# sloisel/MultiGridBarrier.jl

Hardware: AMD Instinct MI355X
Metric: Newton iters/sec + wall-clock to converge, 2D P2 p-Laplace L=9 (higher is better)
Workload: dtype f64

## Files before the change

### multigridbarrier.jl_amd/csrc/mf_big_inv.hpp

```cpp
#pragma once
#include "mf_device.hpp"
#include "mf_big_subst.hpp"

namespace mgbhip {
namespace {

constexpr int BIGI_THREADS = 1024;

#include "ldlt32.hpp"

__device__ __forceinline__ void block_ldlt32(double (*Dn)[NB + 1], double* dq, int nb, int tid, int32_t* __restrict__ status) {
    block_ldlt32_mfma(Dn, dq, nb, tid, status);
}
__device__ __forceinline__ void block_inverse32_sel(const double (*Ls)[NB + 1], double (*Wv)[NB + 1], double (*Tm)[17], int tid) {
    block_inverse32_mfma(Ls, Wv, Tm, tid);
}

__device__ __forceinline__ void slice_transform(double (*P)[ST + 1], double (*Pout)[ST + 1], double (*P2)[ST + 1],
                                                const double (*Wv)[NB + 1], const double* rd, int lane, int wave) {
    const int fr = lane & 15, fk = lane >> 4;
    const int rr = 16 * wave + fr;
    double4_t acc0 = {0.0, 0.0, 0.0, 0.0}, acc1 = {0.0, 0.0, 0.0, 0.0};
#pragma unroll
    for (int kk = 0; kk < NB / 4; ++kk) {
        const double a = P[4 * kk + fk][rr];
        if (kk < 4) acc0 = __builtin_amdgcn_mfma_f64_16x16x4f64(Wv[fr][4 * kk + fk], a, acc0, 0, 0, 0);
        acc1 = __builtin_amdgcn_mfma_f64_16x16x4f64(Wv[16 + fr][4 * kk + fk], a, acc1, 0, 0, 0);
    }
#pragma unroll
    for (int r = 0; r < 4; ++r) {
        const int q0 = fk + 4 * r, q1 = 16 + fk + 4 * r;
        Pout[q0][rr] = acc0[r];
        Pout[q1][rr] = acc1[r];
        if (P2) {
            P2[q0][rr] = acc0[r] * rd[q0];
            P2[q1][rr] = acc1[r] * rd[q1];
        }
    }
}

#ifdef MGB_STEP_PROBE
#define PROBE(i) do { __builtin_amdgcn_sched_barrier(0); __builtin_amdgcn_s_waitcnt(0); if (is_la && blockIdx.y == 0 && tid == 0 && j0 == 64 && gridDim.y == 1 && F.k > 400) g_probe[i] = wall_clock64(); if (!is_la && blockIdx.x == 0 && blockIdx.y == 0 && tid == 0 && j0 == 64 && gridDim.y == 1 && F.k > 400) g_probe[16 + i] = wall_clock64(); __builtin_amdgcn_s_waitcnt(0); __builtin_amdgcn_sched_barrier(0); } while (0)
#else
#define PROBE(i) do { } while (0)
#endif

__global__ __launch_bounds__(256, 3) void mf_big_step(const FrontDev* __restrict__ fr, int32_t first, int j0,
                                                   double* __restrict__ arena, double* __restrict__ dscr,
                                                   double* __restrict__ dvec, int32_t* __restrict__ status,
                                                   int do_diag) {
    __shared__ double Wv[NB][NB + 1];
    __shared__ double Dn[NB][NB + 1];
    __shared__ double Tm[16][17];
    __shared__ double dq[NB], rdq[NB];
    __shared__ double Pa[NB][ST + 1];
    __shared__ double Pb[NB][ST + 1];
    const FrontDev F = fr[first + blockIdx.y];
    const int m = F.m, k = F.k;
    if (j0 >= k) return;
    const int nb = min(NB, k - j0);
    const int j1 = j0 + nb;
    const int T = (m - j1 + ST - 1) / ST;
    const int tid = threadIdx.x, lane = tid & 63, wave = tid >> 6;
    double* W = arena + F.F_off;
    double* slot = dscr + ((int64_t)blockIdx.y * 2 + ((j0 / NB) & 1)) * (NB * NB);
    const bool is_la = blockIdx.x == gridDim.x - 1;
    int ti = 0, tj = 0;
    if (!is_la) {
        const int lin = blockIdx.x;
        ti = (int)((sqrt(8.0 * lin + 1.0) - 1.0) * 0.5);
        while ((ti + 1) * (ti + 2) / 2 <= lin) ++ti;
        while (ti * (ti + 1) / 2 > lin) --ti;
        tj = lin - ti * (ti + 1) / 2;
        if (ti >= T) return;
    }
    const bool look = j1 < k;
    const int nbn = look ? min(NB, k - j1) : 0;
    const int rbase = is_la ? j1 : j1 + ti * ST, cbase = j1 + tj * ST;
    PROBE(0);
#ifdef MGB_STEP_PROBE
    if (is_la && blockIdx.y == 0 && tid == 0 && j0 == 64 && gridDim.y == 1 && F.k > 400) g_probe[34] = clock64();
#endif
    const int fr16 = lane & 15, fk = lane >> 4;

    double pa[NB * ST / 256], pb[NB * ST / 256];
#pragma unroll
    for (int u = 0; u < NB * ST / 256; ++u) {
        const int i = tid + 256 * u, rr = i % ST, q = i / ST;
        const int r = rbase + rr, c = cbase + rr;
        const bool rin = is_la ? (rr < nbn) : (r < m);
        pa[u] = (q < nb && rin) ? W[r + (int64_t)(j0 + q) * m] : 0.0;
        pb[u] = (!is_la && ti != tj && q < nb && c < m) ? W[c + (int64_t)(j0 + q) * m] : 0.0;
    }
    double cw[4][4];
    if (!is_la) {
#pragma unroll
        for (int tb = 0; tb < 4; ++tb)
#pragma unroll
            for (int r = 0; r < 4; ++r) {
                const int row = rbase + 16 * wave + fr16, col = cbase + 16 * tb + fk + 4 * r;
                cw[tb][r] = (row < m && col < m && row >= col) ? W[row + (int64_t)col * m] : 0.0;
            }
    } else {
#pragma unroll
        for (int t = 0; t < 4; ++t) {
            const int i = tid + 256 * t, rr = i % NB, c = i / NB;
            cw[0][t] = (look && rr >= c && rr < nbn) ? W[(j1 + rr) + (int64_t)(j1 + c) * m] : 0.0;
        }
    }
    if (do_diag) {
        for (int i = tid; i < NB * NB; i += 256) {
            const int rr = i % NB, c = i / NB;
            Dn[rr][c] = (rr >= c && rr < nb) ? W[(j0 + rr) + (int64_t)(j0 + c) * m] : 0.0;
        }
        __syncthreads();
        block_ldlt32(Dn, dq, nb, tid, is_la ? status : nullptr);
        block_inverse32_sel(Dn, Wv, Tm, tid);
    } else {
        for (int i = tid; i < NB * NB; i += 256) {
            const int rr = i % NB, c = i / NB;
            const double v = (rr >= c && rr < nb) ? slot[rr + NB * c] : 0.0;
            Wv[rr][c] = (rr > c) ? v : (rr == c ? 1.0 : 0.0);
            if (rr == c) dq[rr] = (rr < nb) ? v : 1.0;
        }
    }
#pragma unroll
    for (int u = 0; u < NB * ST / 256; ++u) {
        const int i = tid + 256 * u, rr = i % ST, q = i / ST;
        Pa[q][rr] = pa[u];
        Pb[q][rr] = pb[u];
    }
    __syncthreads();
    PROBE(1);
    if (tid < NB) rdq[tid] = 1.0 / dq[tid];
    if (is_la ? T == 0 : blockIdx.x == 0) {
        {
            const int rt = wave & 1, ct = wave >> 1;
            if (ct <= rt) {
                double4_t accm = {0.0, 0.0, 0.0, 0.0};
#pragma unroll
                for (int kk = 0; kk < NB / 4; ++kk) {
                    const int kq = 4 * kk + fk;
                    accm = __builtin_amdgcn_mfma_f64_16x16x4f64(kq < nb ? Wv[kq][16 * ct + fr16] / dq[kq] : 0.0, Wv[kq][16 * rt + fr16], accm, 0, 0, 0);
                }
#pragma unroll
                for (int r = 0; r < 4; ++r) {
                    const int row = 16 * rt + fr16, col = 16 * ct + fk + 4 * r;
                    if (row < nb && col < row) W[(j0 + col) + (int64_t)(j0 + row) * m] = accm[r];
                    else if (row < nb && col == row) dvec[F.idx_off + j0 + row] = accm[r];
                }
            }
        }
    }
    if (is_la && !look) return;
    __syncthreads();
    PROBE(2);
    if (is_la) {
        if (wave < 2) slice_transform(Pa, Pa, Pb, Wv, rdq, lane, wave);
        __syncthreads();
        PROBE(3);
        {
            const int rt = wave & 1, ct = wave >> 1;
            double4_t accd = {0.0, 0.0, 0.0, 0.0};
#pragma unroll
            for (int kk = 0; kk < NB / 4; ++kk)
                accd = __builtin_amdgcn_mfma_f64_16x16x4f64(Pb[4 * kk + fk][16 * ct + fr16], Pa[4 * kk + fk][16 * rt + fr16],
                                                            accd, 0, 0, 0);
#pragma unroll
            for (int r = 0; r < 4; ++r) {
                const int rr = 16 * rt + fr16, c = 16 * ct + fk + 4 * r;
                Dn[rr][c] = -accd[r];
            }
        }
        __syncthreads();
#pragma unroll
        for (int t = 0; t < 4; ++t) {
            const int i = tid + 256 * t, rr = i % NB, c = i / NB;
            Dn[rr][c] = (rr >= c && rr < nbn) ? cw[0][t] + Dn[rr][c] : 0.0;
        }
        __syncthreads();
        double* nslot = dscr + ((int64_t)blockIdx.y * 2 + ((j1 / NB) & 1)) * (NB * NB);
        PROBE(4);
#ifdef MGB_STEP_PROBE
        double sv[4];
        for (int t = 0; t < 4; ++t) { const int i = tid + 256 * t; sv[t] = Dn[i % NB][i / NB]; }
        __syncthreads();
        __builtin_amdgcn_sched_barrier(0);
        if (is_la && blockIdx.y == 0 && tid == 0 && j0 == 64 && gridDim.y == 1 && F.k > 400) { g_probe[32] = clock64(); g_probe[36] = wall_clock64(); }
        __builtin_amdgcn_sched_barrier(0);
        block_ldlt32(Dn, dq, nbn, tid, nullptr);
        __builtin_amdgcn_sched_barrier(0);
        if (is_la && blockIdx.y == 0 && tid == 0 && j0 == 64 && gridDim.y == 1 && F.k > 400) { g_probe[33] = clock64(); g_probe[37] = wall_clock64(); }
        __builtin_amdgcn_sched_barrier(0);
        for (int t = 0; t < 4; ++t) { const int i = tid + 256 * t; Dn[i % NB][i / NB] = sv[t]; }
        __syncthreads();
        __builtin_amdgcn_sched_barrier(0);
        if (is_la && blockIdx.y == 0 && tid == 0 && j0 == 64 && gridDim.y == 1 && F.k > 400) { g_probe[38] = clock64(); g_probe[44] = wall_clock64(); }
        __builtin_amdgcn_sched_barrier(0);
#endif
        block_ldlt32(Dn, dq, nbn, tid, status);
#ifdef MGB_STEP_PROBE
        __builtin_amdgcn_sched_barrier(0);
        if (is_la && blockIdx.y == 0 && tid == 0 && j0 == 64 && gridDim.y == 1 && F.k > 400) { g_probe[39] = clock64(); g_probe[45] = wall_clock64(); }
        __builtin_amdgcn_sched_barrier(0);
#endif
        PROBE(5);
        block_inverse32_sel(Dn, Wv, Tm, tid);
        PROBE(6);
        for (int i = tid; i < NB * NB; i += 256) {
            const int rr = i % NB, c = i / NB;
            if (rr >= c && rr < nbn) nslot[rr + NB * c] = (rr == c) ? dq[rr] : Wv[rr][c];
        }
        PROBE(7);
#ifdef MGB_STEP_PROBE
        if (is_la && blockIdx.y == 0 && tid == 0 && j0 == 64 && gridDim.y == 1 && F.k > 400) g_probe[35] = clock64();
#endif
        return;
    }
    if (ti == tj) {
        slice_transform(Pa, Pa, Pb, Wv, rdq, lane, wave);
    } else {
        slice_transform(Pa, Pa, nullptr, Wv, rdq, lane, wave);
        {
            const int rr = 16 * wave + fr16;
            double4_t acc0 = {0.0, 0.0, 0.0, 0.0}, acc1 = {0.0, 0.0, 0.0, 0.0};
#pragma unroll
            for (int kk = 0; kk < NB / 4; ++kk) {
                const double a = Pb[4 * kk + fk][rr];
                if (kk < 4) acc0 = __builtin_amdgcn_mfma_f64_16x16x4f64(Wv[fr16][4 * kk + fk], a, acc0, 0, 0, 0);
                acc1 = __builtin_amdgcn_mfma_f64_16x16x4f64(Wv[16 + fr16][4 * kk + fk], a, acc1, 0, 0, 0);
            }
#pragma unroll
            for (int r = 0; r < 4; ++r) {
                const int q0 = fk + 4 * r, q1 = 16 + fk + 4 * r;
                Pb[q0][rr] = acc0[r] * rdq[q0];
                Pb[q1][rr] = acc1[r] * rdq[q1];
            }
        }
    }
    __syncthreads();
    PROBE(3);
    double4_t acc[4];
#pragma unroll
    for (int tb = 0; tb < 4; ++tb) acc[tb] = double4_t{0.0, 0.0, 0.0, 0.0};
#pragma unroll
    for (int kk = 0; kk < NB / 4; ++kk) {
        const double s = Pa[4 * kk + fk][16 * wave + fr16];
#pragma unroll
        for (int tb = 0; tb < 4; ++tb) {
            if (ti == tj && tb > wave) continue;
            acc[tb] = __builtin_amdgcn_mfma_f64_16x16x4f64(Pb[4 * kk + fk][16 * tb + fr16], s, acc[tb], 0, 0, 0);
        }
    }
    const int nskip = (blockIdx.x == 0 && look) ? nbn : 0;
#pragma unroll
    for (int tb = 0; tb < 4; ++tb)
#pragma unroll
        for (int r = 0; r < 4; ++r) {
            const int row = rbase + 16 * wave + fr16, col = cbase + 16 * tb + fk + 4 * r;
            if (row < m && col < m && row >= col && !(row - j1 < nskip && col - j1 < nskip))
                W[row + (int64_t)col * m] = cw[tb][r] - acc[tb][r];
        }
    PROBE(4);
}

__global__ __launch_bounds__(256) void mf_tri_pack(int m, const double* __restrict__ F, double* __restrict__ packed, int unpack,
                                                   double* __restrict__ Fout) {
    const int c = blockIdx.x;
    if (c >= m) return;
    const int64_t base = (int64_t)c * m - ((int64_t)c * (c - 1)) / 2;
    for (int r = c + threadIdx.x; r < m; r += 256) {
        if (unpack) Fout[r + (int64_t)c * m] = packed[base + (r - c)];
        else packed[base + (r - c)] = F[r + (int64_t)c * m];
    }
}

__global__ __launch_bounds__(256) void mf_big_diag0(const FrontDev* __restrict__ fr, int32_t first,
                                                    const double* __restrict__ arena, double* __restrict__ dscr,
                                                    int32_t* __restrict__ status) {
    __shared__ double Wv[NB][NB + 1];
    __shared__ double Dn[NB][NB + 1];
    __shared__ double Tm[16][17];
    __shared__ double dq[NB];
    const FrontDev F = fr[first + blockIdx.x];
    const int m = F.m, nb = min(NB, F.k), tid = threadIdx.x;
    const double* W = arena + F.F_off;
    for (int i = tid; i < NB * NB; i += 256) {
        const int rr = i % NB, c = i / NB;
        Dn[rr][c] = (rr >= c && rr < nb) ? W[rr + (int64_t)c * m] : 0.0;
    }
    __syncthreads();
    block_ldlt32(Dn, dq, nb, tid, status);
    block_inverse32_sel(Dn, Wv, Tm, tid);
    double* slot = dscr + (int64_t)blockIdx.x * 2 * (NB * NB);
    for (int i = tid; i < NB * NB; i += 256) {
        const int rr = i % NB, c = i / NB;
        if (rr >= c && rr < nb) slot[rr + NB * c] = (rr == c) ? dq[rr] : Wv[rr][c];
    }
}

__global__ __launch_bounds__(256) void mf_big_gather(const FrontDev* __restrict__ fr, int32_t first,
                                                     const GatherRec* __restrict__ grec, const int32_t* __restrict__ gmap,
                                                     const int32_t* __restrict__ a_src,
                                                     const int32_t* __restrict__ a_dst,
                                                     const int32_t* __restrict__ a_colptr,
                                                     const double* __restrict__ Hval, double* __restrict__ arena,
                                                     double* __restrict__ dscr, int32_t* __restrict__ status, int with_diag,
                                                     int ct ) {
    const FrontDev F = fr[first + blockIdx.y];
    const GatherRec G = grec[blockIdx.y];
    const int m = F.m;
    const int32_t* mp = gmap + G.map_off;
    if (with_diag && blockIdx.x == gridDim.x - 1) {
        __shared__ double Wv[NB][NB + 1];
        __shared__ double Dn[NB][NB + 1];
        __shared__ double Tm[16][17];
// ... 517 lines not shown
                for (int t = 0; t < 4; ++t) v += pa[ps][t].a * zr[2 * t] + pa[ps][t].b * zr[2 * t + 1];
                v += quad_perm_f64<0xB1>(v);
                v += quad_perm_f64<0x4E>(v);
                if (cp == 0) gl[q] += v;
            }
        }
        for (int q = cq + 2 * CPP; q - cq < j0; q += CPP) {
            const double* Aq = Fm + (int64_t)min(q, j0 - 1) * m + j0 + 2 * cp;
            D2 a[4];
#pragma unroll
            for (int t = 0; t < 4; ++t) {
                if (nb == NB) a[t] = *reinterpret_cast<const D2*>(Aq + 8 * t);
                else {
                    const int o = 2 * cp + 8 * t;
                    a[t].a = Aq[min(o, nb - 1) - 2 * cp];
                    a[t].b = Aq[min(o + 1, nb - 1) - 2 * cp];
                }
            }
            double v = 0.0;
#pragma unroll
            for (int t = 0; t < 4; ++t) v += a[t].a * zr[2 * t] + a[t].b * zr[2 * t + 1];
            v += quad_perm_f64<0xB1>(v);
            v += quad_perm_f64<0x4E>(v);
            if (cp == 0 && q < j0) gl[q] += v;
        }
        if (j0 == 256) BP(7);
        __syncthreads();
    }
    BP(9);
}

inline void launch_big_assemble(const FactorArgs& a, const MfLaunch& L, bool with_diag) {
    if (big_assembly_kind(L) != MF_ASM_GATHER) {
        launch_big_assemble_cols(a, L);
        return;
    }
    if (a.grec) {
        const int ct = big_gather_ct(L, a.gather_ct);
        const dim3 ga((L.max_m + ct - 1) / ct + (with_diag ? 1 : 0), L.count);
        hipLaunchKernelGGL(mf_big_gather, ga, dim3(256), big_gather_lds(L), a.st, a.fr, L.first, a.grec + L.grec_first, a.gmap,
                           a.a_src, a.a_dst, a.a_colptr, a.values, a.arena, a.dscr, a.status, with_diag ? 1 : 0, ct);
        return;
    }
    dim3 ga = big_assemble_grid(L);
    const int ct = CT;
    if (with_diag) ga.x += 1;
    hipLaunchKernelGGL(mf_big_gather_lds, ga, dim3(256), big_gather_lds(L), a.st, a.fr, L.first, a.children, a.rel, a.a_src, a.a_dst,
                       a.a_colptr, a.values, a.arena, L.max_m, a.dscr, a.status, with_diag ? 1 : 0, ct);
}

inline void launch_big_diag0(const FactorArgs& a, const MfLaunch& L, int nfronts) {
    hipLaunchKernelGGL(mf_big_diag0, dim3(nfronts), dim3(256), 0, a.st, a.fr, L.first, a.arena, a.dscr, a.status);
}
inline void launch_inv_steps(const FactorArgs& a, const MfLaunch& L, int nfronts, bool diag_in_step0) {
    for (int j0 = 0; j0 < L.max_k; j0 += NB) {
        const int rem = L.max_m - j0;
        const int T = std::max(0, (rem - 1 + ST - 1) / ST);
        const dim3 gs(T * (T + 1) / 2 + 1, nfronts);
        hipLaunchKernelGGL(mf_big_step, gs, dim3(256), 0, a.st, a.fr, L.first, j0, a.arena, a.dscr, a.dvec, a.status,
                           (j0 == 0 && diag_in_step0) ? 1 : 0);
    }
}

inline void launch_tri_pack(int m, double* F, double* packed, bool unpack, hipStream_t st) {
    hipLaunchKernelGGL(mf_tri_pack, dim3(m), dim3(256), 0, st, m, unpack ? (const double*)nullptr : F, packed, unpack ? 1 : 0,
                       unpack ? F : (double*)nullptr);
}

inline size_t fwd_inv_lds(int max_m) {
    return (size_t)(((max_m + 1) & ~1) + NB * (NB + 1) + 2 * NB + BIGI_THREADS) * sizeof(double);
}
inline size_t bwd_inv_lds(int max_m, int max_k) {
    return (size_t)(((max_m + 1) & ~1) + ((max_k + 1) & ~1) + NB * (NB + 1) + 2 * NB + (max_m + 1) / 2) * sizeof(double);
}
inline void launch_fwd_inv(const SolveArgs& a, const MfLaunch& L) {
    hipLaunchKernelGGL(mf_fwd_inv, dim3(L.count), dim3(BIGI_THREADS), fwd_inv_lds(L.max_m), a.st, a.fr, L.first, a.front_idx,
                       a.ug_ptr, a.ug_src, a.arena, a.dvec, a.b, a.y, a.uvec);
}
inline void launch_bwd_inv(const SolveArgs& a, const MfLaunch& L) {
    hipLaunchKernelGGL(mf_bwd_inv, dim3(L.count), dim3(BIGI_THREADS), bwd_inv_lds(L.max_m, L.max_k), a.st, a.fr, L.first,
                       a.front_idx, a.arena, a.dvec, a.y, a.x);
}

}
}
```

### multigridbarrier.jl_amd/csrc/mf_launch_plan.hpp

```cpp
#pragma once
#include <algorithm>
#include <cstdint>
#include <cstdlib>
#include <vector>

#include "mf_analysis.hpp"

namespace mgbhip {

struct MfLaunch {
    int32_t first, count;
    int32_t cls;
    int32_t max_m, max_k;
    int32_t max_child = 0;
    bool tiny = false;
    bool wave = false;
    bool inv = false;
    bool iface = false;
    int32_t grec_first = -1;
};

constexpr int BIG_INV_MAX_M = 7000;
constexpr int GATHER_MAX_CHILD = 8;
constexpr int BIG_DIAG0_MIN_COUNT = 24;

struct MfSwitches {
    bool no_geo;
    bool old_big;
    bool merge_groups;
    bool packed_leaves;
    bool wave_small;
    int64_t inv_min_n;
    int64_t wave_min_n;
    bool gather_lds_maps;
    int gather_ct;
    static MfSwitches from_env() {
        auto on = [](const char* name) { const char* e = getenv(name); return e && e[0] == '1'; };
        auto num = [](const char* name, long long dflt) { const char* e = getenv(name); return e ? atoll(e) : dflt; };
        return {on("MGBHIP_NO_GEO"), on("MGBHIP_OLD_BIG"), !on("MGBHIP_NO_MERGE_GROUPS"), !on("MGBHIP_NO_PACKED_LEAVES"),
                !on("MGBHIP_NO_WAVE_SMALL"), num("MGBHIP_INV_MIN_N", 1024), num("MGBHIP_WAVE_MIN_N", 0),
                on("MGBHIP_GATHER_LDS_MAPS"), (int)num("MGBHIP_GATHER_CT", 0)};
    }
};

using LevelLaunches = std::vector<std::vector<MfLaunch>>;

inline MfLaunch launch_of_range(const MfPlan& plan, MfLaunch L, int32_t first, int32_t count) {
    L.first = first; L.count = count;
    L.max_m = 0; L.max_k = 0; L.max_child = 0;
    for (int32_t t = first; t < first + count; ++t) {
        L.max_m = std::max(L.max_m, plan.fronts[t].m);
        L.max_k = std::max(L.max_k, plan.fronts[t].k);
        L.max_child = std::max(L.max_child, plan.fronts[t].nchild);
    }
    return L;
}

inline void merge_straggler_groups(const MfPlan& plan, std::vector<MfLaunch>& G) {
    auto absorb = [&](size_t into, size_t from) {
        MfLaunch& A = G[into];
        const MfLaunch& B = G[from];
        A.first = B.first;
        A.count += B.count;
        A.max_k = std::max(A.max_k, B.max_k);
        A.max_child = std::max(A.max_child, B.max_child);
        G.erase(G.begin() + (long)from);
    };
    if (G.size() >= 2 && G.back().cls == 0 && G.back().inv) {
        int64_t lds_count = 0;
        bool ok = true;
        for (size_t g = 0; g + 1 < G.size(); ++g) { lds_count += G[g].count; ok = ok && !G[g].tiny && plan.fronts[G[g].first].m > 32; }
        if (ok && lds_count <= G.back().count)
            while (G.size() >= 2) absorb(G.size() - 1, G.size() - 2);
    }
    for (size_t g = 0; g + 1 < G.size();) {
        const bool next_lds = G[g + 1].cls != 0;
        if (next_lds && !G[g].tiny && (G[g].count < 256 || 4 * (int64_t)G[g].count < G[g + 1].count)) absorb(g + 1, g);
        else ++g;
    }
}

inline void split_interface_front(const MfPlan& plan, LevelLaunches& levels, bool inv_allowed) {
    const int32_t q = plan.iface_front;
    for (auto& G : levels) {
        for (size_t g = 0; g < G.size(); ++g) {
            const MfLaunch L = G[g];
            if (q < L.first || q >= L.first + L.count) continue;
            std::vector<MfLaunch> out;
            if (q > L.first) out.push_back(launch_of_range(plan, L, L.first, q - L.first));
            MfLaunch I = launch_of_range(plan, L, q, 1);
            I.cls = 0; I.tiny = false; I.wave = false; I.iface = true;
            I.inv = (I.max_m <= BIG_INV_MAX_M && inv_allowed);
            out.push_back(I);
            if (q + 1 < L.first + L.count) out.push_back(launch_of_range(plan, L, q + 1, L.first + L.count - q - 1));
// ... 99 lines not shown
inline MfAssembly big_assembly_kind(const MfLaunch& L) {
    if (L.cls) return MF_ASM_NONE;
    if (L.max_child < 1 || L.max_child > GATHER_MAX_CHILD || big_gather_lds(L) > 40 * 1024) return MF_ASM_COLS;
    return MF_ASM_GATHER;
}
inline MfBlock0 big_block0_kind(const MfLaunch& L, bool inv) {
    if (L.cls || !inv) return MF_B0_NA;
    if (!L.iface && big_assembly_kind(L) == MF_ASM_GATHER) return MF_B0_GATHER;
    return (L.iface || L.count >= BIG_DIAG0_MIN_COUNT) ? MF_B0_DIAG0 : MF_B0_STEP0;
}
inline int backward_small_kmax(const MfLaunch& L) { return L.max_k <= 8 ? 8 : (L.max_k <= 16 ? 16 : 0); }

constexpr int GATHER_MIN_WGS = 768;
inline int big_gather_ct(const MfLaunch& L, int forced) {
    if (forced == 8 || forced == 16 || forced == 32) return forced;
    int ct = 8;
    while (ct < 32 && (int64_t)L.count * ((L.max_m + 2 * ct - 1) / (2 * ct)) >= GATHER_MIN_WGS) ct *= 2;
    return ct;
}

struct GatherRec {
    int64_t map_off;
    int64_t base[GATHER_MAX_CHILD];
    int32_t ld[GATHER_MAX_CHILD];
    int32_t bs[GATHER_MAX_CHILD];
};

inline void build_gather_maps(const MfPlan& plan, LevelLaunches& levels, std::vector<GatherRec>& recs, std::vector<int32_t>& gmap) {
    recs.clear();
    gmap.clear();
    for (auto& lev : levels)
        for (auto& L : lev) {
            L.grec_first = -1;
            if (L.count == 0 || big_assembly_kind(L) != MF_ASM_GATHER) continue;
            L.grec_first = (int32_t)recs.size();
            for (int32_t q = L.first; q < L.first + L.count; ++q) {
                const Front& f = plan.fronts[q];
                GatherRec R{};
                R.map_off = (int64_t)gmap.size();
                gmap.resize(gmap.size() + (size_t)f.nchild * (size_t)f.m, -1);
                for (int32_t c = 0; c < f.nchild; ++c) {
                    const Front& ch = plan.fronts[plan.children[f.child_off + c]];
                    R.base[c] = ch.F_off + (int64_t)ch.k * ch.m + ch.k;
                    R.ld[c] = ch.m;
                    R.bs[c] = ch.m - ch.k;
                    int32_t* mp = gmap.data() + R.map_off + (int64_t)c * f.m;
                    for (int32_t j = 0; j < ch.m - ch.k; ++j) mp[plan.rel[ch.rel_off + j]] = j;
                }
                recs.push_back(R);
            }
        }
}

constexpr int MF_LAUNCH_ROW = 16;
inline int64_t launch_rows(const LevelLaunches& levels, const LevelLaunches& solves, bool leaf_packed, bool robust,
                           int32_t* out, int64_t cap) {
    int64_t n = 0;
    for (size_t l = 0; l < levels.size(); ++l) {
        int32_t bwd = 0;
        for (auto& S : solves[l])
            if (S.cls && !S.tiny) { const int km = backward_small_kmax(S); bwd = km == 8 ? MF_BWD_K8 : (km == 16 ? MF_BWD_K16 : MF_BWD_GENERAL); }
        for (auto& L : levels[l]) {
            if (n < cap && out) {
                const bool inv = L.inv && !robust;
                int32_t* r = out + n * MF_LAUNCH_ROW;
                r[0] = (int32_t)l; r[1] = L.first; r[2] = L.count; r[3] = L.cls; r[4] = L.max_m; r[5] = L.max_k; r[6] = L.max_child;
                r[7] = L.tiny; r[8] = L.wave; r[9] = inv; r[10] = L.iface; r[11] = L.tiny && leaf_packed;
                r[12] = big_assembly_kind(L); r[13] = big_block0_kind(L, inv); r[14] = (L.cls && !L.tiny) ? bwd : (int32_t)MF_BWD_NA; r[15] = 0;
            }
            ++n;
        }
    }
    return n;
}

}
```

### multigridbarrier.jl_amd/csrc/mf_numeric.hip

```cpp
#include <hip/hip_runtime.h>

#include <cstdio>

#include <algorithm>
#include <cstdlib>

#include "../../include/mgbhip.h"
#include "mf_solver.hpp"
#include "mf_device.hpp"
#include "mf_small.hpp"
#include "mf_big_subst.hpp"
#include "mf_big_inv.hpp"

namespace mgbhip {

namespace {

int32_t query_lds_cap() {
    if (hipFuncSetAttribute((const void*)mf_factor_small<8, true>, hipFuncAttributeMaxDynamicSharedMemorySize,
                            (int)factor_small_lds(128)) == hipSuccess)
        return 128;
    (void)hipGetLastError();
    return 88;
}
// ... 108 lines not shown
        const double one = 1.0;
        d_one.upload(&one, 1, st);
        MGB_HIP_CHECK(hipStreamSynchronize(st));
    }
    d_tbig.alloc(plan.front_idx.size() ? plan.front_idx.size() : 1);
    d_tsol.alloc(plan.front_idx.size() ? plan.front_idx.size() : 1);
    d_dvec.alloc(plan.front_idx.size() ? plan.front_idx.size() : 1);
    d_status.alloc(2);
    d_status.zero(st);
}

void MfSolver::analyze(int64_t n, const int32_t* rowptr, const int32_t* colidx, hipStream_t st,
                       const double* coords, int dim, bool protect_peeled, const int32_t* top, int64_t ntop) {
    const MfSwitches sw = MfSwitches::from_env();
    MfOptions opt;
    opt.protect_peeled = protect_peeled;
    opt.top = top;
    opt.ntop = ntop;
    opt.border = true;
    mf_analyze(n, rowptr, colidx, opt, plan, sw.no_geo ? nullptr : coords, dim);
    const int32_t nf = (int32_t)plan.fronts.size();
    std::vector<FrontDev> fd(nf);
    for (int32_t i = 0; i < nf; ++i) {
        const Front& f = plan.fronts[i];
        fd[i] = FrontDev{f.k, f.m, f.nchild, f.a_cnt, f.F_off, f.idx_off, f.u_off, f.child_off, f.rel_off, f.a_off, f.acol_off, -1, 0, 0};
    }
    upload_plan(st);

    lds_cap = query_lds_cap();
    const bool inv_ok = !sw.old_big && query_inv_optin();
    level_launches = classify_launches(plan, lds_cap, inv_ok, sw);
    level_solves = merge_level_solves(level_launches);
    uses_inv = false;
    const std::vector<char> on_big_path = fronts_on_big_path(plan, level_launches);
    int32_t max_big = 1;
    for (auto& lev : level_launches)
        for (auto& L : lev) {
            uses_inv = uses_inv || L.inv;
            if (!L.cls) max_big = std::max(max_big, L.count);
        }
    d_dscr.alloc((size_t)max_big * 2 * NB * NB);

    std::vector<int64_t> ug_ptr, ug_src;
    build_gather_lists(plan, on_big_path, fd, ug_ptr, ug_src);
    leaf_packed = sw.packed_leaves && pack_leaf_fronts(plan, level_launches, on_big_path, fd);
    d_ug_ptr.upload(ug_ptr, st);
    d_ug_src.upload(ug_src, st);
    std::vector<GatherRec> grec;
    std::vector<int32_t> gmap;
    if (!sw.gather_lds_maps) build_gather_maps(plan, level_launches, grec, gmap);
    gather_ct = sw.gather_ct;
    if (grec.empty()) { d_grec.release(); d_gmap.release(); }
    else { d_grec.upload(grec, st); d_gmap.upload(gmap, st); }
    d_fronts.upload(fd, st);
    h_fronts = fd;
    h_a_dst = remap_a_dst(plan, level_launches);
    d_a_dst.upload(h_a_dst, st);
    if (const char* e = getenv("MGBHIP_DEBUG"); e && atoi(e) >= 2) dump_plan(plan, level_launches);
    analyzed = true;
    MGB_HIP_CHECK(hipStreamSynchronize(st));
}

void MfSolver::set_direct_map(const int32_t* value_map, int64_t nnz, int64_t tail_base, hipStream_t st) {
    std::vector<int32_t> as(plan.a_src.size());
    for (size_t t = 0; t < as.size(); ++t) {
        const int64_t src = plan.a_src[t];
        const int64_t v = src < nnz ? (int64_t)value_map[src] : tail_base + (src - nnz);
        MGB_REQUIRE(v < (int64_t)INT32_MAX, "direct value index exceeds 32 bits");
        as[t] = (int32_t)v;
    }
    d_a_src_direct.upload(as, st);
    MGB_HIP_CHECK(hipStreamSynchronize(st));
}

void MfSolver::factor(const double* d_values, hipStream_t st, StageTimers* timers, bool direct, bool condensed) {
    MGB_REQUIRE(!direct || d_a_src_direct.n > 0, "MfSolver::factor: no direct value map");
    MGB_REQUIRE(!condensed || (direct && condensed_ok), "MfSolver::factor: condensed leaves are not enabled");
    MGB_REQUIRE(analyzed, "MfSolver::factor before analyze");
    const FactorArgs a{condensed ? d_fronts_c.p : d_fronts.p, d_children.p, d_rel.p,
                       condensed ? d_a_src_c.p : (direct ? d_a_src_direct.p : d_a_src.p), condensed ? d_a_dst_c.p : d_a_dst.p,
                       condensed ? d_a_colptr_c.p : d_a_colptr.p, d_values, d_arena.p, d_dscr.p, d_dvec.p, d_status.p, st,
                       d_grec.n ? d_grec.p : nullptr, d_gmap.p, gather_ct};
    if (timers) timers->begin("factor");
    factored_inv = !robust;
    if (!status_zero) MGB_HIP_CHECK(hipMemsetAsync(d_status.p, 0, sizeof(int32_t), st));
    status_zero = false;
    factored_condensed = condensed;
    int lvno = -1;
    for (auto& lev : level_launches) {
        LevelScope lvscope(timers, "fac", ++lvno);
        for (auto& L : lev) {
            if (L.count == 0) continue;
            if (condensed && lvno == 0) continue;
            if (L.tiny) launch_factor_tiny(a, L);
            else if (L.wave && L.cls <= 32) launch_factor_wave<32>(a, L);
            else if (L.wave) launch_factor_wave<48>(a, L);
            else if (L.cls) launch_factor_small(a, L);
            else {
                const bool inv = L.inv && !robust;
                const MfBlock0 b0 = big_block0_kind(L, inv);
                MGB_REQUIRE(!L.iface || (bool)iface_reduce, "MfSolver: interface front without a reduction hook");
                launch_big_assemble(a, L, b0 == MF_B0_GATHER);
                if (L.iface) {
                    const Front& fi = plan.fronts[L.first];
                    const int64_t tri = (int64_t)fi.m * (fi.m + 1) / 2;
                    d_ifpack.ensure((size_t)tri);
                    launch_tri_pack(fi.m, d_arena.p + fi.F_off, d_ifpack.p, false, st);
                    iface_reduce(d_ifpack.p, tri);
                    launch_tri_pack(fi.m, d_arena.p + fi.F_off, d_ifpack.p, true, st);
                }
                if (inv) {
                    if (b0 == MF_B0_DIAG0) launch_big_diag0(a, L, L.count);
                    launch_inv_steps(a, L, L.count, b0 == MF_B0_STEP0);
                } else
                    launch_subst_steps(a, L, L.count);
            }
        }
    }
    MGB_HIP_CHECK(hipGetLastError());
    if (timers) timers->end();
}

void MfSolver::solve(const double* d_b, double* d_x, hipStream_t st, StageTimers* timers) {
    MGB_REQUIRE(analyzed, "MfSolver::solve before analyze");
    if (timers) timers->begin("trisolve");
    const size_t n = (size_t)plan.n;
    MGB_HIP_CHECK(hipMemcpyAsync(d_bx.p, d_b, n * sizeof(double), hipMemcpyDeviceToDevice, st));
    MGB_HIP_CHECK(hipMemsetAsync(d_bx.p + n, 0, sizeof(double), st));
    forward_pass(d_bx.p, st, timers);
    backward_pass(d_xx.p, st, timers);
    MGB_HIP_CHECK(hipMemcpyAsync(d_x, d_xx.p, n * sizeof(double), hipMemcpyDeviceToDevice, st));
    MGB_HIP_CHECK(hipGetLastError());
    if (timers) timers->end();
}

void MfSolver::solve_border(double* d_x_np1, hipStream_t st, StageTimers* timers) {
    MGB_REQUIRE(analyzed, "MfSolver::solve_border before analyze");
    if (timers) timers->begin("trisolve");
    const size_t n = (size_t)plan.n;
    if (!y_zero) {
        MGB_HIP_CHECK(hipMemsetAsync(d_y.p, 0, n * sizeof(double), st));
        y_zero = true;
    }
    if (!y_border_one) {
        MGB_HIP_CHECK(hipMemcpyAsync(d_y.p + n, d_one.p, sizeof(double), hipMemcpyDeviceToDevice, st));
        y_border_one = true;
    }
    backward_pass(d_x_np1, st, timers);
    MGB_HIP_CHECK(hipGetLastError());
    if (timers) timers->end();
}

void MfSolver::forward_pass(const double* d_b, hipStream_t st, StageTimers* timers) {
    y_border_one = false;
    y_zero = false;
    const SolveArgs a = solve_args(d_b, nullptr, st);
    int lvno = -1;
    for (auto& lev : level_solves) {
        LevelScope lvscope(timers, "fwd", ++lvno);
        for (auto& L : lev) {
            if (L.count == 0) continue;
            if (L.tiny) launch_forward_tiny(a, L);
            else if (L.cls) launch_forward_small(a, L);
            else if (L.inv && factored_inv) launch_fwd_inv(a, L);
            else if (L.max_m <= BIG1_MAX_M) launch_fwd_big1(a, L);
            else launch_fwd_big_steps(a, L);
// ... 144 lines not shown
```

### multigridbarrier.jl_amd/csrc/mf_solver.hpp

```cpp
#pragma once
#include <functional>

#include "common.hpp"
#include "mf_analysis.hpp"
#include "mf_launch_plan.hpp"
#include "kernels.hpp"

namespace mgbhip {

struct FrontDev {
    int32_t k, m, nchild, a_cnt;
    int64_t F_off, idx_off, u_off, child_off, rel_off, a_off, acol_off;
    int64_t ug_off;
    int32_t packed;
    int32_t pad_;
};

struct FactorArgs {
    const FrontDev* fr;
    const int32_t *children, *rel, *a_src, *a_dst, *a_colptr;
    const double* values;
    double *arena, *dscr, *dvec;
    int32_t* status;
    hipStream_t st;
    const GatherRec* grec;
    const int32_t* gmap;
    int gather_ct;
};
struct SolveArgs {
    const FrontDev* fr;
    const int32_t *front_idx, *children, *rel;
    const int64_t *ug_ptr, *ug_src;
    const double *arena, *dvec;
    const double* b;
    double *y, *x, *uvec, *tbig, *tsol;
    hipStream_t st;
};

class MfSolver {
   public:
    MfPlan plan;
    void analyze(int64_t n, const int32_t* rowptr, const int32_t* colidx, hipStream_t st,
                 const double* coords = nullptr, int dim = 0, bool protect_peeled = false,
                 const int32_t* top = nullptr, int64_t ntop = 0);
    std::function<void(double*, int64_t)> iface_reduce;
    void factor(const double* d_values, hipStream_t st, StageTimers* timers, bool direct = false, bool condensed = false);
    bool enable_condensed(int64_t N, int P, const int32_t* ucol, int64_t slack0, int64_t nnz, int64_t tail_base, hipStream_t st);
    bool condensed_ready() const { return condensed_ok; }
    bool leaves_packed() const { return leaf_packed; }
    const LeafDesc* leaf_desc() const { return d_leaf_desc.p; }
    double* arena() { return d_arena.p; }
    int32_t* leaf_status() { return d_status.p + 1; }
    const int32_t* status_flags() const { return d_status.p; }
    int32_t* status_flags_rw() { return d_status.p; }
    void flags_cleared() { status_zero = true; leaf_zero = true; }
    bool leaf_flag_zero() const { return leaf_zero; }
    void leaf_flag_used() { leaf_zero = false; }
    void set_direct_map(const int32_t* value_map, int64_t nnz, int64_t tail_base, hipStream_t st);
    bool has_direct_map() const { return d_a_src_direct.n > 0; }
    void solve(const double* d_b, double* d_x, hipStream_t st, StageTimers* timers);
    void solve_border(double* d_x_np1, hipStream_t st, StageTimers* timers);
    void chain_stats(double* out8) const;
    int64_t launches(int32_t* out, int64_t cap) const;
    int status(hipStream_t st);
    void status_async(int32_t* h_dst, hipStream_t st) const;
    static int status_from(const int32_t* flags2, bool with_leaves) {
        return (flags2[0] || (with_leaves && flags2[1])) ? MGBHIP_ERR_NOT_SPD : MGBHIP_OK;
    }
    bool factored_condensed = false;
    bool analyzed = false;
    bool robust = false;
    bool has_inverse_path() const { return uses_inv; }
    bool factored_inv = false;

   private:
    void upload_plan(hipStream_t st);
    SolveArgs solve_args(const double* d_b, double* d_x, hipStream_t st) const {
        return {d_fronts.p, d_front_idx.p, d_children.p, d_rel.p, d_ug_ptr.p, d_ug_src.p, d_arena.p, d_dvec.p, d_b, d_y.p, d_x,
                d_uvec.p, d_tbig.p, d_tsol.p, st};
    }
    void forward_pass(const double* d_b_np1, hipStream_t st, StageTimers* timers);
    void backward_pass(double* d_x_np1, hipStream_t st, StageTimers* timers);
    DevBuf<double> d_bx, d_xx, d_one;
    DevBuf<FrontDev> d_fronts;
    DevBuf<int32_t> d_front_idx, d_children, d_rel, d_a_src, d_a_src_direct, d_a_dst, d_a_colptr;
    DevBuf<GatherRec> d_grec;
    DevBuf<int32_t> d_gmap;
    DevBuf<int64_t> d_ug_ptr, d_ug_src;
    DevBuf<double> d_arena, d_uvec, d_y, d_tbig, d_tsol, d_dscr, d_dvec;
    DevBuf<double> d_ifpack;
    DevBuf<int32_t> d_status;
    bool condensed_ok = false;
    bool leaf_packed = false;
    std::vector<FrontDev> h_fronts;
    std::vector<int32_t> h_a_dst;
    DevBuf<FrontDev> d_fronts_c;
    DevBuf<int32_t> d_a_src_c, d_a_dst_c, d_a_colptr_c;
    DevBuf<LeafDesc> d_leaf_desc;
    std::vector<std::vector<MfLaunch>> level_launches;
    std::vector<std::vector<MfLaunch>> level_solves;
    int gather_ct = 0;
    int32_t lds_cap = 88;
    bool uses_inv = false;
    bool y_border_one = false;
    bool y_zero = false;
    bool status_zero = false, leaf_zero = false;
};

}
```

Baseline: 683.6.

## Precompute compact per-step work items and strip multiple column tiles per block

Replaces the dense 2D grid of the blocked-inverse step kernel (max-front triangle times front count, with early-exit blocks) with a host-built list of work items covering only the real tiles of each front. When there are enough items, each block processes a strip of up to four adjacent column tiles, reusing the transformed row panel in shared memory and reloading only the column panel and C tile. Items are sorted so longer strips launch first. This cuts idle blocks and repeated row-panel transforms, at the cost of less parallelism per launch and extra syncs inside the strip loop.

```diff
diff --git a/multigridbarrier.jl_amd/csrc/mf_big_inv.hpp b/multigridbarrier.jl_amd/csrc/mf_big_inv.hpp
--- a/multigridbarrier.jl_amd/csrc/mf_big_inv.hpp
+++ b/multigridbarrier.jl_amd/csrc/mf_big_inv.hpp
@@ -40,46 +40,45 @@
 }
 
 #ifdef MGB_STEP_PROBE
-#define PROBE(i) do { __builtin_amdgcn_sched_barrier(0); __builtin_amdgcn_s_waitcnt(0); if (is_la && blockIdx.y == 0 && tid == 0 && j0 == 64 && gridDim.y == 1 && F.k > 400) g_probe[i] = wall_clock64(); if (!is_la && blockIdx.x == 0 && blockIdx.y == 0 && tid == 0 && j0 == 64 && gridDim.y == 1 && F.k > 400) g_probe[16 + i] = wall_clock64(); __builtin_amdgcn_s_waitcnt(0); __builtin_amdgcn_sched_barrier(0); } while (0)
+#define PROBE(i) do { __builtin_amdgcn_sched_barrier(0); __builtin_amdgcn_s_waitcnt(0); if (is_la && fo == 0 && tid == 0 && j0 == 64 && solo && F.k > 400) g_probe[i] = wall_clock64(); if (!is_la && ti == 0 && tj0 == 0 && fo == 0 && tid == 0 && j0 == 64 && solo && F.k > 400) g_probe[16 + i] = wall_clock64(); __builtin_amdgcn_s_waitcnt(0); __builtin_amdgcn_sched_barrier(0); } while (0)
 #else
 #define PROBE(i) do { } while (0)
 #endif
 
-__global__ __launch_bounds__(256, 3) void mf_big_step(const FrontDev* __restrict__ fr, int32_t first, int j0,
+static_assert(STEP_NB == NB && STEP_ST == ST, "the step items are laid out for this panel width and tile edge");
+__global__ __launch_bounds__(256, 3) void mf_big_step(const FrontDev* __restrict__ fr, const StepItem* __restrict__ items,
+                                                   int32_t first, int j0, int do_diag,
                                                    double* __restrict__ arena, double* __restrict__ dscr,
-                                                   double* __restrict__ dvec, int32_t* __restrict__ status,
-                                                   int do_diag) {
+                                                   double* __restrict__ dvec, int32_t* __restrict__ status) {
     __shared__ double Wv[NB][NB + 1];
     __shared__ double Dn[NB][NB + 1];
     __shared__ double Tm[16][17];
     __shared__ double dq[NB], rdq[NB];
     __shared__ double Pa[NB][ST + 1];
     __shared__ double Pb[NB][ST + 1];
-    const FrontDev F = fr[first + blockIdx.y];
+    const StepItem it = items[blockIdx.x];
+    const int fo = it.front();
+    const FrontDev F = fr[first + fo];
     const int m = F.m, k = F.k;
-    if (j0 >= k) return;
     const int nb = min(NB, k - j0);
     const int j1 = j0 + nb;
     const int T = (m - j1 + ST - 1) / ST;
     const int tid = threadIdx.x, lane = tid & 63, wave = tid >> 6;
     double* W = arena + F.F_off;
-    double* slot = dscr + ((int64_t)blockIdx.y * 2 + ((j0 / NB) & 1)) * (NB * NB);
-    const bool is_la = blockIdx.x == gridDim.x - 1;
-    int ti = 0, tj = 0;
-    if (!is_la) {
-        const int lin = blockIdx.x;
-        ti = (int)((sqrt(8.0 * lin + 1.0) - 1.0) * 0.5);
-        while ((ti + 1) * (ti + 2) / 2 <= lin) ++ti;
-        while (ti * (ti + 1) / 2 > lin) --ti;
-        tj = lin - ti * (ti + 1) / 2;
-        if (ti >= T) return;
-    }
+    double* slot = dscr + ((int64_t)fo * 2 + ((j0 / NB) & 1)) * (NB * NB);
+    const bool is_la = (it.kind() & STEP_ITEM_LOOK) != 0;
+    const int ti = it.ti, tj0 = it.tj0, ntile = it.n();
+#ifdef MGB_STEP_PROBE
+    const bool solo = (it.kind() & STEP_ITEM_SOLO) != 0;
+#endif
+    int tj = tj0;
     const bool look = j1 < k;
     const int nbn = look ? min(NB, k - j1) : 0;
-    const int rbase = is_la ? j1 : j1 + ti * ST, cbase = j1 + tj * ST;
+    const int rbase = is_la ? j1 : j1 + ti * ST;
+    int cbase = j1 + tj * ST;
     PROBE(0);
 #ifdef MGB_STEP_PROBE
-    if (is_la && blockIdx.y == 0 && tid == 0 && j0 == 64 && gridDim.y == 1 && F.k > 400) g_probe[34] = clock64();
+    if (is_la && fo == 0 && tid == 0 && j0 == 64 && solo && F.k > 400) g_probe[34] = clock64();
 #endif
     const int fr16 = lane & 15, fk = lane >> 4;
 
@@ -114,7 +113,7 @@
             Dn[rr][c] = (rr >= c && rr < nb) ? W[(j0 + rr) + (int64_t)(j0 + c) * m] : 0.0;
         }
         __syncthreads();
-        block_ldlt32(Dn, dq, nb, tid, is_la ? status : nullptr);
+        block_ldlt32(Dn, dq, nb, tid, (is_la || (!look && ti == 0 && tj0 == 0)) ? status : nullptr);
         block_inverse32_sel(Dn, Wv, Tm, tid);
     } else {
         for (int i = tid; i < NB * NB; i += 256) {
@@ -133,7 +132,7 @@
     __syncthreads();
     PROBE(1);
     if (tid < NB) rdq[tid] = 1.0 / dq[tid];
-    if (is_la ? T == 0 : blockIdx.x == 0) {
+    if (is_la ? T == 0 : (ti == 0 && tj0 == 0)) {
         {
             const int rt = wave & 1, ct = wave >> 1;
             if (ct <= rt) {
@@ -179,29 +178,29 @@
             Dn[rr][c] = (rr >= c && rr < nbn) ? cw[0][t] + Dn[rr][c] : 0.0;
         }
         __syncthreads();
-        double* nslot = dscr + ((int64_t)blockIdx.y * 2 + ((j1 / NB) & 1)) * (NB * NB);
+        double* nslot = dscr + ((int64_t)fo * 2 + ((j1 / NB) & 1)) * (NB * NB);
         PROBE(4);
 #ifdef MGB_STEP_PROBE
         double sv[4];
         for (int t = 0; t < 4; ++t) { const int i = tid + 256 * t; sv[t] = Dn[i % NB][i / NB]; }
         __syncthreads();
         __builtin_amdgcn_sched_barrier(0);
-        if (is_la && blockIdx.y == 0 && tid == 0 && j0 == 64 && gridDim.y == 1 && F.k > 400) { g_probe[32] = clock64(); g_probe[36] = wall_clock64(); }
+        if (is_la && fo == 0 && tid == 0 && j0 == 64 && solo && F.k > 400) { g_probe[32] = clock64(); g_probe[36] = wall_clock64(); }
         __builtin_amdgcn_sched_barrier(0);
         block_ldlt32(Dn, dq, nbn, tid, nullptr);
         __builtin_amdgcn_sched_barrier(0);
-        if (is_la && blockIdx.y == 0 && tid == 0 && j0 == 64 && gridDim.y == 1 && F.k > 400) { g_probe[33] = clock64(); g_probe[37] = wall_clock64(); }
+        if (is_la && fo == 0 && tid == 0 && j0 == 64 && solo && F.k > 400) { g_probe[33] = clock64(); g_probe[37] = wall_clock64(); }
         __builtin_amdgcn_sched_barrier(0);
         for (int t = 0; t < 4; ++t) { const int i = tid + 256 * t; Dn[i % NB][i / NB] = sv[t]; }
         __syncthreads();
         __builtin_amdgcn_sched_barrier(0);
-        if (is_la && blockIdx.y == 0 && tid == 0 && j0 == 64 && gridDim.y == 1 && F.k > 400) { g_probe[38] = clock64(); g_probe[44] = wall_clock64(); }
+        if (is_la && fo == 0 && tid == 0 && j0 == 64 && solo && F.k > 400) { g_probe[38] = clock64(); g_probe[44] = wall_clock64(); }
         __builtin_amdgcn_sched_barrier(0);
 #endif
         block_ldlt32(Dn, dq, nbn, tid, status);
 #ifdef MGB_STEP_PROBE
         __builtin_amdgcn_sched_barrier(0);
-        if (is_la && blockIdx.y == 0 && tid == 0 && j0 == 64 && gridDim.y == 1 && F.k > 400) { g_probe[39] = clock64(); g_probe[45] = wall_clock64(); }
+        if (is_la && fo == 0 && tid == 0 && j0 == 64 && solo && F.k > 400) { g_probe[39] = clock64(); g_probe[45] = wall_clock64(); }
         __builtin_amdgcn_sched_barrier(0);
 #endif
         PROBE(5);
@@ -213,15 +212,14 @@
         }
         PROBE(7);
 #ifdef MGB_STEP_PROBE
-        if (is_la && blockIdx.y == 0 && tid == 0 && j0 == 64 && gridDim.y == 1 && F.k > 400) g_probe[35] = clock64();
+        if (is_la && fo == 0 && tid == 0 && j0 == 64 && solo && F.k > 400) g_probe[35] = clock64();
 #endif
         return;
     }
-    if (ti == tj) {
-        slice_transform(Pa, Pa, Pb, Wv, rdq, lane, wave);
-    } else {
-        slice_transform(Pa, Pa, nullptr, Wv, rdq, lane, wave);
-        {
+    if (ti == tj) slice_transform(Pa, Pa, Pb, Wv, rdq, lane, wave);
+    else slice_transform(Pa, Pa, nullptr, Wv, rdq, lane, wave);
+    auto tile = [&]() __attribute__((always_inline)) {
+        if (ti != tj) {
             const int rr = 16 * wave + fr16;
             double4_t acc0 = {0.0, 0.0, 0.0, 0.0}, acc1 = {0.0, 0.0, 0.0, 0.0};
 #pragma unroll
@@ -237,31 +235,58 @@
                 Pb[q1][rr] = acc1[r] * rdq[q1];
             }
         }
-    }
-    __syncthreads();
-    PROBE(3);
-    double4_t acc[4];
-#pragma unroll
-    for (int tb = 0; tb < 4; ++tb) acc[tb] = double4_t{0.0, 0.0, 0.0, 0.0};
-#pragma unroll
-    for (int kk = 0; kk < NB / 4; ++kk) {
-        const double s = Pa[4 * kk + fk][16 * wave + fr16];
-#pragma unroll
-        for (int tb = 0; tb < 4; ++tb) {
-            if (ti == tj && tb > wave) continue;
-            acc[tb] = __builtin_amdgcn_mfma_f64_16x16x4f64(Pb[4 * kk + fk][16 * tb + fr16], s, acc[tb], 0, 0, 0);
-        }
-    }
-    const int nskip = (blockIdx.x == 0 && look) ? nbn : 0;
-#pragma unroll
-    for (int tb = 0; tb < 4; ++tb)
-#pragma unroll
-        for (int r = 0; r < 4; ++r) {
-            const int row = rbase + 16 * wave + fr16, col = cbase + 16 * tb + fk + 4 * r;
-            if (row < m && col < m && row >= col && !(row - j1 < nskip && col - j1 < nskip))
-                W[row + (int64_t)col * m] = cw[tb][r] - acc[tb][r];
-        }
-    PROBE(4);
+        __syncthreads();
+        PROBE(3);
+        double4_t acc[4];
+#pragma unroll
+        for (int tb = 0; tb < 4; ++tb) acc[tb] = double4_t{0.0, 0.0, 0.0, 0.0};
+#pragma unroll
+        for (int kk = 0; kk < NB / 4; ++kk) {
+            const double s = Pa[4 * kk + fk][16 * wave + fr16];
+#pragma unroll
+            for (int tb = 0; tb < 4; ++tb) {
+                if (ti == tj && tb > wave) continue;
+                acc[tb] = __builtin_amdgcn_mfma_f64_16x16x4f64(Pb[4 * kk + fk][16 * tb + fr16], s, acc[tb], 0, 0, 0);
+            }
+        }
+        const int nskip = (ti == 0 && tj == 0 && look) ? nbn : 0;
+#pragma unroll
+        for (int tb = 0; tb < 4; ++tb)
+#pragma unroll
+            for (int r = 0; r < 4; ++r) {
+                const int row = rbase + 16 * wave + fr16, col = cbase + 16 * tb + fk + 4 * r;
+                if (row < m && col < m && row >= col && !(row - j1 < nskip && col - j1 < nskip))
+                    W[row + (int64_t)col * m] = cw[tb][r] - acc[tb][r];
+            }
+        PROBE(4);
+    };
+    tile();
+    for (int t = 1; t < ntile; ++t) {
+        ++tj;
+        cbase += ST;
+        __syncthreads();
+        int ltid = tid;
+        asm volatile("" : "+v"(ltid));
+#pragma unroll
+        for (int u = 0; u < NB * ST / 256; ++u) {
+            const int i = ltid + 256 * u, rr = i % ST, q = i / ST;
+            const int c = cbase + rr;
+            if (ti == tj) Pb[q][rr] = Pa[q][rr] * rdq[q];
+            else Pb[q][rr] = (q < nb && c < m) ? W[c + (int64_t)(j0 + q) * m] : 0.0;
+        }
+        {
+            const int lrow = rbase + 16 * (ltid >> 6) + (ltid & 15), lfk = (ltid & 63) >> 4;
+#pragma unroll
+            for (int tb = 0; tb < 4; ++tb)
+#pragma unroll
+                for (int r = 0; r < 4; ++r) {
+                    const int col = cbase + 16 * tb + lfk + 4 * r;
+                    cw[tb][r] = (lrow < m && col < m && lrow >= col) ? W[lrow + (int64_t)col * m] : 0.0;
+                }
+        }
+        __syncthreads();
+        tile();
+    }
 }
 
 __global__ __launch_bounds__(256) void mf_tri_pack(int m, const double* __restrict__ F, double* __restrict__ packed, int unpack,
@@ -885,13 +910,12 @@
 inline void launch_big_diag0(const FactorArgs& a, const MfLaunch& L, int nfronts) {
     hipLaunchKernelGGL(mf_big_diag0, dim3(nfronts), dim3(256), 0, a.st, a.fr, L.first, a.arena, a.dscr, a.status);
 }
-inline void launch_inv_steps(const FactorArgs& a, const MfLaunch& L, int nfronts, bool diag_in_step0) {
+inline void launch_inv_steps(const FactorArgs& a, const MfLaunch& L, bool diag_in_step0) {
     for (int j0 = 0; j0 < L.max_k; j0 += NB) {
-        const int rem = L.max_m - j0;
-        const int T = std::max(0, (rem - 1 + ST - 1) / ST);
-        const dim3 gs(T * (T + 1) / 2 + 1, nfronts);
-        hipLaunchKernelGGL(mf_big_step, gs, dim3(256), 0, a.st, a.fr, L.first, j0, a.arena, a.dscr, a.dvec, a.status,
-                           (j0 == 0 && diag_in_step0) ? 1 : 0);
+        const StepRange R = a.step_tab[L.step_first + j0 / NB];
+        if (R.count == 0) continue;
+        hipLaunchKernelGGL(mf_big_step, dim3(R.count), dim3(256), 0, a.st, a.fr, a.sitems + R.off, L.first, j0,
+                           (j0 == 0 && diag_in_step0) ? 1 : 0, a.arena, a.dscr, a.dvec, a.status);
     }
 }
 
diff --git a/multigridbarrier.jl_amd/csrc/mf_launch_plan.hpp b/multigridbarrier.jl_amd/csrc/mf_launch_plan.hpp
--- a/multigridbarrier.jl_amd/csrc/mf_launch_plan.hpp
+++ b/multigridbarrier.jl_amd/csrc/mf_launch_plan.hpp
@@ -2,6 +2,7 @@
 #include <algorithm>
 #include <cstdint>
 #include <cstdlib>
+#include <stdexcept>
 #include <vector>
 
 #include "mf_analysis.hpp"
@@ -18,6 +19,7 @@
     bool inv = false;
     bool iface = false;
     int32_t grec_first = -1;
+    int32_t step_first = -1;
 };
 
 constexpr int BIG_INV_MAX_M = 7000;
@@ -34,12 +36,13 @@
     int64_t wave_min_n;
     bool gather_lds_maps;
     int gather_ct;
+    int step_strip;
     static MfSwitches from_env() {
         auto on = [](const char* name) { const char* e = getenv(name); return e && e[0] == '1'; };
         auto num = [](const char* name, long long dflt) { const char* e = getenv(name); return e ? atoll(e) : dflt; };
         return {on("MGBHIP_NO_GEO"), on("MGBHIP_OLD_BIG"), !on("MGBHIP_NO_MERGE_GROUPS"), !on("MGBHIP_NO_PACKED_LEAVES"),
                 !on("MGBHIP_NO_WAVE_SMALL"), num("MGBHIP_INV_MIN_N", 1024), num("MGBHIP_WAVE_MIN_N", 0),
-                on("MGBHIP_GATHER_LDS_MAPS"), (int)num("MGBHIP_GATHER_CT", 0)};
+                on("MGBHIP_GATHER_LDS_MAPS"), (int)num("MGBHIP_GATHER_CT", 0), (int)num("MGBHIP_STEP_STRIP", 0)};
     }
 };
 
@@ -245,6 +248,75 @@
         }
 }
 
+constexpr int STEP_NB = 32;
+constexpr int STEP_ST = 64;
+constexpr int STEP_MAX_STRIP = 4;
+constexpr uint32_t STEP_ITEM_LOOK = 1;
+constexpr uint32_t STEP_ITEM_SOLO = 2;
+struct StepItem {
+    uint32_t w;
+    uint16_t ti, tj0;
+    static StepItem make(int32_t front, int n, uint32_t kind, int ti, int tj0) {
+        return {(uint32_t)front | ((uint32_t)n << 24) | (kind << 28), (uint16_t)ti, (uint16_t)tj0};
+    }
+    constexpr int32_t front() const { return (int32_t)(w & 0xFFFFFFu); }
+    constexpr int n() const { return (int)((w >> 24) & 15u); }
+    constexpr uint32_t kind() const { return w >> 28; }
+};
+static_assert(sizeof(StepItem) == 8, "a step item is 8 bytes");
+struct StepRange { int32_t off, count; };
+
+inline int step_tile_rows(int m, int k, int j0) {
+    const int j1 = j0 + std::min(STEP_NB, k - j0);
+    return (m - j1 + STEP_ST - 1) / STEP_ST;
+}
+inline int64_t step_strip_count(int T, int g) {
+    int64_t s = 0;
+    for (int ti = 0; ti < T; ++ti) s += (ti + g) / g;
+    return s;
+}
+constexpr int STEP_MIN_ITEMS = 768;
+inline int big_step_strip(const MfLaunch& L, int j0, int forced) {
+    if (forced == 1 || forced == 2 || forced == 4) return forced;
+    const int T = std::max(0, step_tile_rows(L.max_m, std::max(L.max_k, j0 + 1), j0));
+    int g = 1;
+    while (g < STEP_MAX_STRIP && (int64_t)L.count * step_strip_count(T, 2 * g) >= STEP_MIN_ITEMS) g *= 2;
+    return g;
+}
+
+inline void build_step_items(const MfPlan& plan, LevelLaunches& levels, int forced, std::vector<StepRange>& tab,
+                             std::vector<StepItem>& items) {
+    tab.clear();
+    items.clear();
+    std::vector<StepItem> tiles;
+    for (auto& lev : levels)
+        for (auto& L : lev) {
+            L.step_first = -1;
+            if (L.count == 0 || L.cls || !L.inv) continue;
+            if (L.count >= (1 << 24)) throw std::length_error("build_step_items: more than 2^24 fronts in one launch");
+            L.step_first = (int32_t)tab.size();
+            const uint32_t solo = L.count == 1 ? STEP_ITEM_SOLO : 0u;
+            for (int j0 = 0; j0 < L.max_k; j0 += STEP_NB) {
+                const int g = big_step_strip(L, j0, forced);
+                const int32_t off = (int32_t)items.size();
+                tiles.clear();
+                for (int32_t q = 0; q < L.count; ++q) {
+                    const Front& f = plan.fronts[L.first + q];
+                    if (j0 >= f.k) continue;
+                    const int T = step_tile_rows(f.m, f.k, j0);
+                    if (j0 + STEP_NB < f.k || T == 0) items.push_back(StepItem::make(q, 0, STEP_ITEM_LOOK | solo, 0, 0));
+                    for (int ti = 0; ti < T; ++ti)
+                        for (int tj0 = 0; tj0 <= ti; tj0 += g)
+                            tiles.push_back(StepItem::make(q, std::min(g, ti + 1 - tj0), solo, ti, tj0));
+                }
+                std::stable_sort(tiles.begin(), tiles.end(), [](const StepItem& a, const StepItem& b) { return a.n() > b.n(); });
+                items.insert(items.end(), tiles.begin(), tiles.end());
+                if (items.size() > (size_t)INT32_MAX) throw std::length_error("build_step_items: more than 2^31 step items");
+                tab.push_back(StepRange{off, (int32_t)items.size() - off});
+            }
+        }
+}
+
 constexpr int MF_LAUNCH_ROW = 16;
 inline int64_t launch_rows(const LevelLaunches& levels, const LevelLaunches& solves, bool leaf_packed, bool robust,
                            int32_t* out, int64_t cap) {
diff --git a/multigridbarrier.jl_amd/csrc/mf_numeric.hip b/multigridbarrier.jl_amd/csrc/mf_numeric.hip
--- a/multigridbarrier.jl_amd/csrc/mf_numeric.hip
+++ b/multigridbarrier.jl_amd/csrc/mf_numeric.hip
@@ -184,6 +184,10 @@
     gather_ct = sw.gather_ct;
     if (grec.empty()) { d_grec.release(); d_gmap.release(); }
     else { d_grec.upload(grec, st); d_gmap.upload(gmap, st); }
+    std::vector<StepItem> sitems;
+    build_step_items(plan, level_launches, sw.step_strip, h_step_tab, sitems);
+    if (sitems.empty()) d_sitems.release();
+    else d_sitems.upload(sitems, st);
     d_fronts.upload(fd, st);
     h_fronts = fd;
     h_a_dst = remap_a_dst(plan, level_launches);
@@ -212,7 +216,7 @@
     const FactorArgs a{condensed ? d_fronts_c.p : d_fronts.p, d_children.p, d_rel.p,
                        condensed ? d_a_src_c.p : (direct ? d_a_src_direct.p : d_a_src.p), condensed ? d_a_dst_c.p : d_a_dst.p,
                        condensed ? d_a_colptr_c.p : d_a_colptr.p, d_values, d_arena.p, d_dscr.p, d_dvec.p, d_status.p, st,
-                       d_grec.n ? d_grec.p : nullptr, d_gmap.p, gather_ct};
+                       d_grec.n ? d_grec.p : nullptr, d_gmap.p, gather_ct, d_sitems.p, h_step_tab.data()};
     if (timers) timers->begin("factor");
     factored_inv = !robust;
     if (!status_zero) MGB_HIP_CHECK(hipMemsetAsync(d_status.p, 0, sizeof(int32_t), st));
@@ -243,7 +247,7 @@
                 }
                 if (inv) {
                     if (b0 == MF_B0_DIAG0) launch_big_diag0(a, L, L.count);
-                    launch_inv_steps(a, L, L.count, b0 == MF_B0_STEP0);
+                    launch_inv_steps(a, L, b0 == MF_B0_STEP0);
                 } else
                     launch_subst_steps(a, L, L.count);
             }
diff --git a/multigridbarrier.jl_amd/csrc/mf_solver.hpp b/multigridbarrier.jl_amd/csrc/mf_solver.hpp
--- a/multigridbarrier.jl_amd/csrc/mf_solver.hpp
+++ b/multigridbarrier.jl_amd/csrc/mf_solver.hpp
@@ -26,6 +26,8 @@
     const GatherRec* grec;
     const int32_t* gmap;
     int gather_ct;
+    const StepItem* sitems;
+    const StepRange* step_tab;
 };
 struct SolveArgs {
     const FrontDev* fr;
@@ -86,6 +88,8 @@
     DevBuf<int32_t> d_front_idx, d_children, d_rel, d_a_src, d_a_src_direct, d_a_dst, d_a_colptr;
     DevBuf<GatherRec> d_grec;
     DevBuf<int32_t> d_gmap;
+    DevBuf<StepItem> d_sitems;
+    std::vector<StepRange> h_step_tab;
     DevBuf<int64_t> d_ug_ptr, d_ug_src;
     DevBuf<double> d_arena, d_uvec, d_y, d_tbig, d_tsol, d_dscr, d_dvec;
     DevBuf<double> d_ifpack;
```

Result: faster. 693.7, median of 6 (+1.5%).
